# AlgoLab/rs-vgaligner

Hardware: AMD Instinct MI355X
Metric: aligned reads/sec (10 kbp ONT vs HLA graph) (higher is better)
Workload: dtype int32+f64

## Files before the change

rs-vgaligner_amd/csrc/vga_poa_t5.hpp:

```cpp
#pragma once

#include "vga_poa_row.hpp"

__device__ __forceinline__ uint64_t t5_uniform64(uint64_t v)
{
    return ((uint64_t)(uint32_t)__builtin_amdgcn_readfirstlane((int)(v >> 32)) << 32) | (uint32_t)__builtin_amdgcn_readfirstlane((int)(uint32_t)v);
}

#define POA_T5_ARGS_OFFSET 40
__device__ __forceinline__ const poa_t5_args *t5_kargs()
{
    uint32_t off = POA_T5_ARGS_OFFSET;
    asm volatile("" : "+s"(off));
    return (const poa_t5_args *)((const char *)__builtin_amdgcn_kernarg_segment_ptr() + off);
}
template <int NT, bool DEF>
__global__ __launch_bounds__(NT) __attribute__((amdgpu_waves_per_eu(5)))
void k_poa_dp_t5(const poa_prob *__restrict__ probs, const char *__restrict__ queries,
                                                       const uint4 *__restrict__ node_tab, const uint32_t *__restrict__ seq32,
                                                       const uint32_t *__restrict__ preds, const poa_t5_args A)
{
    poa_row *rows = A.rows;
    uint8_t *pool_arg = A.pool;
    const uint32_t lds_cols = t5_own(A.lds_cols), hg_cols = t5_own(A.hg_cols), win_mask = t5_own(A.win_mask);
    enum : uint32_t { ST_CHUNKED = 1u, ST_QPLAIN = 2u, ST_FAILED = 4u, ST_PREV_LDS = 8u, ST_PREV_FAR_USE = 16u };
    uint32_t st = (A.cp.n_slots != 0 ? ST_CHUNKED : 0u) | ST_PREV_LDS;
#define chunked ((st & ST_CHUNKED) != 0)
#define failed ((st & ST_FAILED) != 0)
#define q_plain ((st & ST_QPLAIN) != 0)
#define prev_lds ((st & ST_PREV_LDS) != 0)
#define prev_far_use ((st & ST_PREV_FAR_USE) != 0)
    struct { int match, mismatch, o1, e1, o2, e2, banded; } P = {t5_own(A.P.match), t5_own(A.P.mismatch), A.P.o1, A.P.e1, A.P.o2, A.P.e2, t5_own(A.P.banded)};
    constexpr int NW = NT / 64;
    constexpr int STEP = NT * 4;
    extern __shared__ __attribute__((aligned(16))) uint8_t smem[];
    int4 *sX = (int4 *)smem;
    int4 *sRed = sX + 2 * NW;
    int32_t *edgeW = (int32_t *)(sRed + NW);
    int32_t *sSink = edgeW + 4;
    uint64_t *sChunk = (uint64_t *)(sSink + 4);
    constexpr int HDR = (3 * NW + 1 + 1 + 2) * 16;
    int32_t *Hs = (int32_t *)(smem + HDR);
    uint16_t *Gs = (uint16_t *)(smem + HDR + 4ull * hg_cols);
    uint16_t *Qn = (uint16_t *)(smem + HDR + 6ull * hg_cols);
    const int edge_idx = (int)(edgeW - Hs);

    if (threadIdx.x == 0) A.outs[blockIdx.x].t_begin = __builtin_amdgcn_s_memrealtime();
    if (A.prio) __builtin_amdgcn_s_setprio(3);
    const poa_prob pb = probs[blockIdx.x];
    const int tid = threadIdx.x, lane = tid & 63, wv = __builtin_amdgcn_readfirstlane(tid >> 6);
    const int qlen = t5_own((int)pb.qlen);
    const char *query = queries + pb.q0;
    const uint4 *ntab = node_tab + t5_own(pb.node0);
    const uint32_t *plist = preds + t5_own(pb.pred0);
    const uint32_t *seqw = seq32 + t5_own(pb.seq0 >> 2);
    poa_row *R = rows + t5_own(pb.row0);
    const uint32_t n_nodes = t5_own(pb.n_nodes), ring_rows = t5_own(pb.ring_rows);

    uint8_t *pool = pool_arg;
    uint64_t state_lo = 0, state_hi = 0;
    if (chunked) {
        int got = -1;
        if (!(pb.flags & 1u)) {
            if (tid == 0) {
                got = poa_slot_acquire(A.cp.slot_flag, A.cp.n_slots, blockIdx.x);
                sSink[1] = got;
            }
            __syncthreads();
            got = __builtin_amdgcn_readfirstlane(sSink[1]);
        }
        if (got < 0) {
            if (tid == 0) {
                poa_out &O = A.outs[blockIdx.x];
                O.t_end = O.t_begin; O.cells = 0; O.vcells = 0; O.maxw = 0; O.nops = 0;
                O.score = POA_NEG; O.row = 0; O.status = POA_ST_POOL;
            }
            return;
        }
        __builtin_amdgcn_fence(__ATOMIC_ACQUIRE, "agent");
        pool = nullptr;
        state_lo = (uint64_t)A.cp.state_base + (uint64_t)(uint32_t)got * A.cp.state_size;
        state_hi = state_lo + A.cp.state_size;
    }

    const int o1 = DEF ? 4 : P.o1, e1 = DEF ? 2 : P.e1, o2 = DEF ? 24 : P.o2, e2 = DEF ? 1 : P.e2;
    const int C1 = 4 * (o1 + e1), C2 = 4 * (o2 + e2) + 1;
    const int D1 = 4 * o1, D2 = 4 * o2 + 1;
    const uint32_t g_bias = (uint32_t)(4 * e1 | (4 * e2) << 8) * 0x00010001u;
    const uint32_t e_probe = (uint32_t)((128 - D1) | (128 - D2) << 8) * 0x00010001u;
    const int bw = t5_own((int)pb.w);

    uint32_t own_head = POA_NIL, own_chunks = 0;
    auto alloc = [&](uint64_t &cur, uint32_t &rem, uint32_t bytes_asked, int slot) -> uint64_t {
        const uint32_t bytes = (bytes_asked + 15u) & ~15u;
        if (__builtin_expect(bytes > rem, 0)) {
            if (chunked) {
                if (slot == 0 && bytes <= POA_CHUNK) {
                    const poa_t5_args *ka = t5_kargs();
                    if (tid == 0) {
                        const uint32_t idx = poa_chunk_pop(ka->cp, blockIdx.x);
                        if (idx != POA_NIL) __hip_atomic_store(ka->cp.next + idx, own_head, __ATOMIC_RELAXED, __HIP_MEMORY_SCOPE_AGENT);
                        if (own_chunks == 0) sChunk[3] = idx;
                        sChunk[0] = idx;
                    }
                    __syncthreads();
                    const uint32_t idx = (uint32_t)__builtin_amdgcn_readfirstlane((int)(uint32_t)sChunk[0]);
                    __syncthreads();
                    if (idx == POA_NIL) st |= ST_FAILED;
                    else {
                        own_head = idx;
                        own_chunks++;
                        cur = poa_uniform_u64(poa_chunk_addr(ka->cp, idx));
                        rem = (uint32_t)POA_CHUNK;
                    }
                } else
                    st |= ST_FAILED;
                if (failed) return cur;
            } else {
                const uint64_t need = bytes > POA_CHUNK ? ((uint64_t)bytes + POA_CHUNK - 1) & ~(POA_CHUNK - 1) : POA_CHUNK;
                const poa_t5_args *ka = t5_kargs();
                if (tid == 0) sChunk[slot] = atomicAdd(ka->pool_next, (unsigned long long)need);
                __syncthreads();
                const uint64_t b = t5_uniform64(sChunk[slot]);
                __syncthreads();
                if (b + need > ka->pool_size) st |= ST_FAILED;
                cur = b;
                rem = (uint32_t)need;
            }
        }
        const uint64_t r = cur;
        cur += bytes;
        rem -= bytes;
        return r;
    };

    int non_acgt = 0;
    for (int t = tid; t < (int)(lds_cols / 4); t += NT) {
        uint32_t hw = 0;
#pragma unroll
        for (int k = 0; k < 4; k++) {
            const int j = 4 * t + k;
            uint32_t code = 0;
            if (j >= 1 && j <= qlen) {
                const char ch = query[j - 1];
                code = (ch == 'A' || ch == 'C' || ch == 'G' || ch == 'T') ? 1u << (((uint32_t)ch >> 1) & 3u) : 0u;
                non_acgt |= code == 0;
            }
            hw |= code << (4 * k);
        }
        Qn[t] = (uint16_t)hw;
    }
    if (__builtin_amdgcn_readfirstlane(__syncthreads_or(non_acgt)) == 0) st |= ST_QPLAIN;

    uint64_t dcur = 0, vcur = state_lo, wide_scratch = 0, ring_base = 0;
    uint32_t dend = 0, vendp = (uint32_t)(state_hi - state_lo);
    uint32_t ring_head = 0;
    if (win_mask != 0xFFFFFFFFu) wide_scratch = alloc(vcur, vendp, 2u * 6u * lds_cols, 1);
    {
        const uint64_t maxrow = (6ull * (uint64_t)((qlen + 8) & ~3) + 15ull) & ~15ull;
        if (chunked) {
            ring_base = alloc(vcur, vendp, (uint32_t)(maxrow * (uint64_t)ring_rows), 1);
        } else {
            const uint64_t rb = (maxrow * (uint64_t)ring_rows + POA_CHUNK - 1) & ~(POA_CHUNK - 1);
            if (tid == 0) sChunk[2] = atomicAdd(A.pool_next, (unsigned long long)rb);
            __syncthreads();
            const uint64_t b = t5_uniform64(sChunk[2]);
            if (b + rb > A.pool_size || rb >= (1ull << 32)) st |= ST_FAILED;
            ring_base = b;
        }
    }
    if (tid == 0) { sSink[2] = POA_NEG; sSink[3] = 0; }
    int prev_beg = 0, prev_end = -1;
    uint32_t seq_word = 0, seq_word_idx = 0xFFFFFFFFu;

    for (uint32_t v = 0; v < n_nodes && !failed; v++) {
    const uint4 nt = ntab[v];
    const uint32_t nlen = nt.y & 0xFFFFFFu;
    for (uint32_t tn = 0; tn < nlen && !failed; tn++) {
        asm volatile("" : "+s"(st));
        POA_MARK("row_topo");
        const uint32_t r = nt.x + tn;
        const bool last = tn + 1 == nlen;
        const bool is_sink = last && (nt.z >> 31) != 0;
        const uint32_t ps = nt.w;
        uint32_t gb = 0;
        if (v > 0) {
            const uint32_t bi = r - 1;
            if ((bi & 3u) == 0 || (bi >> 2) != seq_word_idx) { seq_word_idx = bi >> 2; seq_word = seqw[seq_word_idx]; }
            gb = (seq_word >> (8u * (bi & 3u))) & 0xffu;
        }
        const bool simple = r > 0 && prev_lds && (tn > 0 || ((nt.y >> 24) == 1u && ps == r - 1));
        const bool writer = wv == (int)(r % (uint32_t)NW);
        POA_MARK("row_prevmax");
        int prev_lmax = 0, prev_rmax = 0;
        if (r > 0) {
            int4 rw = make_int4(INT32_MIN, INT32_MAX, INT32_MIN, 0);
            if (lane < NW) rw = sRed[lane];
            int b = rw.x, t;
            t = poa_dpp<0x111, 0xf>(INT32_MIN, b); b = t > b ? t : b;
            if (NW > 2) { t = poa_dpp<0x112, 0xf>(INT32_MIN, b); b = t > b ? t : b; }
            if (NW > 4) { t = poa_dpp<0x114, 0xf>(INT32_MIN, b); b = t > b ? t : b; }
            if (NW > 8) { t = poa_dpp<0x118, 0xf>(INT32_MIN, b); b = t > b ? t : b; }
            const int rbest = __builtin_amdgcn_readlane(b, NW - 1);
            const uint64_t tie = __builtin_amdgcn_ballot_w64(rw.x == rbest);
            if (__builtin_expect(__builtin_popcountll(tie) == 1, 1)) {
                const int w1 = __builtin_ctzll(tie);
                prev_lmax = __builtin_amdgcn_readlane(rw.y, w1);
                prev_rmax = __builtin_amdgcn_readlane(rw.z, w1);
            } else {
                int lm = rw.x == rbest ? rw.y : INT32_MAX, rm = rw.x == rbest ? rw.z : INT32_MIN;
                t = poa_dpp<0x111, 0xf>(INT32_MAX, lm); lm = t < lm ? t : lm;
                t = poa_dpp<0x111, 0xf>(INT32_MIN, rm); rm = t > rm ? t : rm;
                if (NW > 2) {
                    t = poa_dpp<0x112, 0xf>(INT32_MAX, lm); lm = t < lm ? t : lm;
                    t = poa_dpp<0x112, 0xf>(INT32_MIN, rm); rm = t > rm ? t : rm;
                }
                if (NW > 4) {
                    t = poa_dpp<0x114, 0xf>(INT32_MAX, lm); lm = t < lm ? t : lm;
                    t = poa_dpp<0x114, 0xf>(INT32_MIN, rm); rm = t > rm ? t : rm;
                }
                if (NW > 8) {
                    t = poa_dpp<0x118, 0xf>(INT32_MAX, lm); lm = t < lm ? t : lm;
                    t = poa_dpp<0x118, 0xf>(INT32_MIN, rm); rm = t > rm ? t : rm;
                }
                prev_lmax = __builtin_amdgcn_readlane(lm, NW - 1);
                prev_rmax = __builtin_amdgcn_readlane(rm, NW - 1);
            }
            if (prev_far_use && writer && lane == 0) { R[r - 1].lmax = prev_lmax; R[r - 1].rmax = prev_rmax; }
        }
        POA_MARK("row_setup");
        const int remain = (int)(nt.z & 0x3fffffffu) + (int)(nlen - 1 - tn);
        int beg, end, np, pbeg = prev_beg, pend = prev_end;
        bool first, single, sp_near;
        uint32_t sp = r - 1;
        uint64_t vpo = 0;
        if (__builtin_expect(simple, 1)) {
            first = tn == 0;
            np = 1; single = true; sp_near = true;
            const int mpl = prev_lmax + 1, mpr = prev_rmax + 1;
            if (!P.banded) { beg = 0; end = qlen; }
            else {
                const int diag = qlen - remain;
                const int lo = mpl < diag ? mpl : diag;
                const int hi = mpr > diag ? mpr : diag;
                beg = lo - bw; if (beg < 0) beg = 0;
                end = hi + bw; if (end > qlen) end = qlen;
            }
        } else {
            first = tn == 0 && v > 0;
            np = v == 0 ? 0 : (tn == 0 ? (int)(nt.y >> 24) : 1);
            bool far = r > 0 && !prev_lds;
            if (first) {
                if (np == 1) far |= ps != r - 1;
                else
                    for (int t = 0; t < np; t++) far |= plist[ps + t] != r - 1;
            }
            single = r > 0 && np == 1;
            sp = first ? ps : r - 1;
            sp_near = sp == r - 1 && prev_lds;
            if (far) __syncthreads();
            int mpl, mpr;
            if (r == 0) { mpl = 0; mpr = 0; }
            else if (!first) { mpl = prev_lmax + 1; mpr = prev_rmax + 1; }
            else {
                mpl = INT32_MAX; mpr = 0;
                for (int t = 0; t < np; t++) {
                    const uint32_t p = np == 1 ? ps : plist[ps + t];
                    int lm, rm;
                    if (p == r - 1) { lm = prev_lmax + 1; rm = prev_rmax + 1; }
                    else {
                        lm = __builtin_amdgcn_readfirstlane(R[p].lmax) + 1;
                        rm = __builtin_amdgcn_readfirstlane(R[p].rmax) + 1;
                    }
                    mpl = lm < mpl ? lm : mpl;
                    mpr = rm > mpr ? rm : mpr;
                }
            }
            if (!P.banded) { beg = 0; end = qlen; }
            else {
                const int diag = qlen - remain;
                const int lo = mpl < diag ? mpl : diag;
                const int hi = mpr > diag ? mpr : diag;
                beg = lo - bw; if (beg < 0) beg = 0;
                end = hi + bw; if (end > qlen) end = qlen;
            }
            if (single && !sp_near) {
                pbeg = __builtin_amdgcn_readfirstlane(R[sp].beg);
                pend = __builtin_amdgcn_readfirstlane(R[sp].end);
                vpo = t5_uniform64(R[sp].voff);
            }
        }
        const int bal = beg & ~3;
        const int W = (end - bal + 1 + 3) & ~3;
        const bool wide = (uint32_t)W + 8u > hg_cols;
        const bool keep = last || wide;
        const uint64_t doff = alloc(dcur, dend, (uint32_t)W * (np > 1 ? 4u : 1u), 0);
        uint64_t voff = 0;
        if (last && !failed) {
            if (r == 0 || (nt.z & 0x40000000u)) voff = chunked ? alloc(dcur, dend, 6u * (uint32_t)W, 0) : alloc(vcur, vendp, 6u * (uint32_t)W, 1);
            else {
                voff = ring_base + (uint64_t)ring_head * ((6u * (uint32_t)((qlen + 8) & ~3) + 15u) & ~15u);
                ring_head = ring_head + 1 == ring_rows ? 0 : ring_head + 1;
            }
        } else if (wide) voff = wide_scratch + (r & 1u) * 6ull * lds_cols;
        if (__builtin_expect(failed, 0)) break;
        if (writer && lane == 0) {
            uint32_t *rec = (uint32_t *)(R + r);
            *(uint4 *)rec = make_uint4((uint32_t)beg, (uint32_t)end, (uint32_t)doff, (uint32_t)(doff >> 32));
            *(uint2 *)(rec + 4) = make_uint2((uint32_t)voff, (uint32_t)(voff >> 32));
            *(HIP_vector_type<uint32_t, 3> *)(rec + 8) = HIP_vector_type<uint32_t, 3>(ps, first ? (uint32_t)np : 0u, keep ? 1u : 0u);
        }
        uint8_t *Vrow = pool + voff;
        uint8_t *drow = pool + doff;
        const uint32_t gd = gb - (uint32_t)'A';
        const bool acgt = gd < 20u && ((0x80045u >> gd) & 1u);
        const int sc_eq = acgt ? P.match : 0, sc_ne = acgt ? -P.mismatch : 0;
        const int gsh = (int)((gb >> 1) & 3u);
        const int ne4t = 4 * sc_ne + 1, mm4 = 4 * (sc_eq - sc_ne);
        const bool staged = !simple && r > 0 && !wide && q_plain;
        if (staged) {
            POA_MARK("row_stage");
            if (chunked) {
                bool no_row = false;
                for (int t = 0; t < np; t++) no_row |= t5_uniform64(R[np == 1 ? sp : plist[ps + t]].voff) == 0;
                if (__builtin_expect(no_row, 0)) st |= ST_FAILED;
            }
            for (int c0 = 0; c0 < W; c0 += STEP) {
                const int c = c0 + 4 * tid;
                const int j0 = bal + c;
                if (j0 <= end && np == 1) {
                    const int bp = __builtin_amdgcn_readfirstlane(R[sp].beg), ep = __builtin_amdgcn_readfirstlane(R[sp].end);
                    const uint64_t vq_off = t5_uniform64(R[sp].voff);
                    const uint8_t *Vq = pool + vq_off;
                    const bool vq_ok = !chunked || vq_off != 0;
                    const int balq = bp & ~3;
                    const int Wq = (ep - balq + 1 + 3) & ~3;
                    const int idx = j0 - balq;
                    int4 hv = make_int4(T4_NEG, T4_NEG, T4_NEG, T4_NEG);
                    uint2 gg = make_uint2(0u, 0u);
                    if (idx >= 0 && idx < Wq && vq_ok) {
                        hv = *(const int4 *)((const int32_t *)Vq + idx);
                        gg = *(const uint2 *)(Vq + 4ll * Wq + 2ll * idx);
                    }
                    const unsigned pspan = (unsigned)(ep - bp);
                    const bool in0 = (unsigned)(j0 - bp) <= pspan, in1 = (unsigned)(j0 + 1 - bp) <= pspan, in2 = (unsigned)(j0 + 2 - bp) <= pspan,
                               in3 = (unsigned)(j0 + 3 - bp) <= pspan;
                    hv.x = in0 ? hv.x : T4_NEG; hv.y = in1 ? hv.y : T4_NEG; hv.z = in2 ? hv.z : T4_NEG; hv.w = in3 ? hv.w : T4_NEG;
                    gg.x = (in0 ? gg.x & 0xffffu : 0u) | (in1 ? gg.x & 0xffff0000u : 0u);
                    gg.y = (in2 ? gg.y & 0xffffu : 0u) | (in3 ? gg.y & 0xffff0000u : 0u);
                    *(int4 *)(Hs + (j0 & win_mask)) = hv;
                    *(uint2 *)(Gs + (j0 & win_mask)) = gg;
                    if (c == 0 && bal > 0) {
                        const int wl = (idx >= 1 && idx - 1 < Wq && vq_ok) ? ((const int32_t *)Vq)[idx - 1] : 0;
                        Hs[(bal - 1) & win_mask] = (unsigned)(j0 - 1 - bp) <= pspan ? wl : T4_NEG;
                    }
                } else if (j0 <= end) {
                    int hm[4], x1[4], x2[4], ah[4], a1[4], a2[4];
                    int hl = T4_NEG, ahl = 0;
#pragma unroll
                    for (int k = 0; k < 4; k++) { hm[k] = T4_NEG; x1[k] = T4_NEG; x2[k] = T4_NEG; ah[k] = 0; a1[k] = 0; a2[k] = 0; }
                    for (int t = 0; t < np; t++) {
                        const uint32_t p = np == 1 ? sp : plist[ps + t];
                        const int bp = __builtin_amdgcn_readfirstlane(R[p].beg), ep = __builtin_amdgcn_readfirstlane(R[p].end);
                        const uint64_t vq_off = t5_uniform64(R[p].voff);
                        const uint8_t *Vq = pool + vq_off;
                        const int balq = bp & ~3;
                        const int Wq = (!chunked || vq_off != 0) ? (ep - balq + 1 + 3) & ~3 : 0;
                        const int idx = j0 - balq;
                        int4 hv = make_int4(0, 0, 0, 0);
                        uint2 gg = make_uint2(0u, 0u);
                        if (idx >= 0 && idx < Wq) {
                            hv = *(const int4 *)((const int32_t *)Vq + idx);
                            gg = *(const uint2 *)(Vq + 4ll * Wq + 2ll * idx);
                        }
                        int wl = (idx >= 1 && idx - 1 < Wq) ? ((const int32_t *)Vq)[idx - 1] : 0;
                        const unsigned pspan = (unsigned)(ep - bp);
                        const int hj[4] = {hv.x, hv.y, hv.z, hv.w};
                        const uint32_t g16[4] = {gg.x & 0xffffu, gg.x >> 16, gg.y & 0xffffu, gg.y >> 16};
#pragma unroll
                        for (int k = 0; k < 4; k++) {
                            if ((unsigned)(j0 + k - bp) <= pspan) {
                                const int h = hj[k], c1 = h - (int)(g16[k] & 255u), c2 = h - (int)(g16[k] >> 8);
                                if (h > hm[k]) { hm[k] = h; ah[k] = t; }
                                if (c1 > x1[k]) { x1[k] = c1; a1[k] = t; }
                                if (c2 > x2[k]) { x2[k] = c2; a2[k] = t; }
                            }
                        }
                        if (j0 >= 1 && (unsigned)(j0 - 1 - bp) <= pspan && wl > hl) { hl = wl; ahl = t; }
                    }
                    const int4 hq = make_int4(hm[0], hm[1], hm[2], hm[3]);
                    uint32_t gv[4];
#pragma unroll
                    for (int k = 0; k < 4; k++) gv[k] = (uint32_t)(hm[k] - x1[k]) | ((uint32_t)(hm[k] - x2[k]) << 8);
                    *(int4 *)(Hs + (j0 & win_mask)) = hq;
                    *(uint2 *)(Gs + (j0 & win_mask)) = make_uint2(gv[0] | (gv[1] << 16), gv[2] | (gv[3] << 16));
                    if (c == 0 && bal > 0) Hs[(bal - 1) & win_mask] = hl;
                    if (np > 1) {
                        *(uint32_t *)(drow + (uint64_t)W + c) = (uint32_t)ahl | ((uint32_t)ah[0] << 8) | ((uint32_t)ah[1] << 16) | ((uint32_t)ah[2] << 24);
                        *(uint32_t *)(drow + 2ull * W + c) = (uint32_t)a1[0] | ((uint32_t)a1[1] << 8) | ((uint32_t)a1[2] << 16) | ((uint32_t)a1[3] << 24);
                        *(uint32_t *)(drow + 3ull * W + c) = (uint32_t)a2[0] | ((uint32_t)a2[1] << 8) | ((uint32_t)a2[2] << 16) | ((uint32_t)a2[3] << 24);
                    }
                }
            }
            POA_LDS_BARRIER();
            pbeg = bal > 0 ? bal - 1 : 0;
            pend = bal + W - 1;
        }
        const uint8_t *Vp = pool + vpo;
        const int balp = pbeg & ~3;

        POA_MARK("row_steps");
        enum : uint32_t { F_SINGLE = 1u, F_NEAR = 2u, F_PLAIN = 4u, F_WIDE = 8u, F_KEEP = 16u, F_SINK = 32u, F_MULTI = 64u, F_SRC = 128u };
        const uint32_t rowf = (single ? F_SINGLE : 0u) | (sp_near ? F_NEAR : 0u) | (q_plain ? F_PLAIN : 0u) | (wide ? F_WIDE : 0u) |
                              (keep ? F_KEEP : 0u) | (is_sink ? F_SINK : 0u) | (np > 1 ? F_MULTI : 0u) | (r == 0 ? F_SRC : 0u);
        int best = INT32_MIN, lpos = beg, rpos = beg;
        const bool hot = (simple || staged) && !wide && q_plain;
        const int rlim = end < pend ? end : pend;
        auto run_steps = [&](auto hot_c) __attribute__((always_inline)) {
        constexpr bool HOT = decltype(hot_c)::value;
        int carry1 = POA_IDENT, carry2 = POA_IDENT, left1 = POA_IDENT, left2 = POA_IDENT;
        int next_left = 0;
        int buf = 0;
        for (int c0 = 0; c0 < W; c0 += STEP, buf ^= 1) {
            uint32_t f = HOT ? (rowf & (F_KEEP | F_SINK)) : rowf;
            asm volatile("" : "+s"(f));
            if (HOT) f |= F_SINGLE | F_NEAR | F_PLAIN;
            const int c = c0 + 4 * tid;
            const int j0 = bal + c;
            const bool lane_act = j0 <= end;
            const int jw0 = bal + c0 + 256 * wv, jw1 = jw0 + 255;
            const bool wave_act = jw0 <= end;
            int d_lp = jw0 - beg, d_rp = rlim - jw1, d_lq = (jw0 > beg ? jw0 : beg) - pbeg - 1;
            asm volatile("" : "+s"(d_lp), "+s"(d_rp), "+s"(d_lq));
            const uint32_t e_lp = (uint32_t)d_lp >> 31;
            const uint32_t e_rp = (uint32_t)d_rp >> 31;
            const uint32_t e_lq = (uint32_t)d_lq >> 31;
            const bool lp = e_lp != 0, rp = e_rp != 0, lq = e_lq != 0;
            int htt[4], ht4[4], e1t[4], e2t[4], pmeta[4];
            int agg1 = POA_IDENT, agg2 = POA_IDENT, alast1 = POA_IDENT, alast2 = POA_IDENT;
#pragma unroll
            for (int k = 0; k < 4; k++) { htt[k] = T4_NEG + 2; ht4[k] = T4_NEG; e1t[k] = T4_NEG + 1; e2t[k] = T4_NEG; pmeta[k] = 0; }
            uint32_t qn = 0u;
            if (wave_act) qn = (uint32_t)Qn[j0 >> 2];
            const bool fastw = HOT ? wave_act
                                   : (f & (F_SINGLE | F_PLAIN)) == (F_SINGLE | F_PLAIN) && wave_act && (!lq || (f & F_NEAR)) && (!rp || ((f & F_NEAR) && end <= pend + 1));
            const int base1 = 4 * e1 * j0, base2 = 4 * e2 * j0;
        if constexpr (HOT) POA_MARK("hot_p1_fast"); else POA_MARK("p1_fast");
            if (__builtin_expect(fastw, 1)) {
                int4 hv;
                uint2 gg;
                int hprev;
                if constexpr (HOT) {
                    hv = *(const int4 *)(Hs + (j0 & win_mask));
                    gg = *(const uint2 *)(Gs + (j0 & win_mask));
                    int left0;
                    if (wv == 0 && c0 > 0) left0 = next_left;
                    else left0 = Hs[(jw0 > 0 ? jw0 - 1 : 0) & (int)win_mask];
                    if (wv == 0 && c0 + STEP < W) next_left = Hs[(jw0 + STEP - 1) & (int)win_mask];
                    hprev = t4_shr1_mov(hv.w, left0);
                } else if (__builtin_expect((f & F_NEAR) != 0, 1)) {
                    hv = *(const int4 *)(Hs + (j0 & win_mask));
                    gg = *(const uint2 *)(Gs + (j0 & win_mask));
                    if (tid == NT - 1) edgeW[buf] = hv.w;
                    {
                        const bool edge = tid == 0 && c0 > 0;
                        int w = Hs[edge ? edge_idx + (buf ^ 1) : ((j0 > 0 ? j0 - 1 : 0) & win_mask)];
                        asm volatile("" : "+v"(w));
                        hprev = w;
                    }
                } else {
                    const int Wp = (pend - balp + 1 + 3) & ~3;
                    const int idx = j0 - balp;
                    hv = *(const int4 *)((const int32_t *)Vp + idx);
                    gg = *(const uint2 *)(Vp + 4ll * Wp + 2ll * idx);
                    hprev = ((const int32_t *)Vp)[idx > 0 ? idx - 1 : 0];
                    asm volatile("" : "+v"(hv.x), "+v"(hv.y), "+v"(hv.z), "+v"(hv.w), "+v"(gg.x), "+v"(gg.y), "+v"(hprev));
                }
                auto phase1 = [&](auto edge_c) {
                    constexpr bool EDGE = decltype(edge_c)::value;
                    int hj[4] = {hv.x, hv.y, hv.z, hv.w};
                    int ga = (int)gg.x, gbb = (int)gg.y;
                    if constexpr (EDGE) {
                        if (rp) {
#pragma unroll
                            for (int k = 0; k < 4; k++) hj[k] = j0 + k > pend ? T4_NEG : hj[k];
                            ga = j0 > pend ? 0 : (j0 + 1 > pend ? (ga & 0xffff) : ga);
                            gbb = j0 + 2 > pend ? 0 : (j0 + 3 > pend ? (gbb & 0xffff) : gbb);
                        }
                        if (lq) {
#pragma unroll
                            for (int k = 0; k < 4; k++) hj[k] = j0 + k < pbeg ? T4_NEG : hj[k];
                            ga = j0 + 1 < pbeg ? 0 : (j0 < pbeg ? (int)((uint32_t)ga & 0xffff0000u) : ga);
                            gbb = j0 + 3 < pbeg ? 0 : (j0 + 2 < pbeg ? (int)((uint32_t)gbb & 0xffff0000u) : gbb);
                        }
                    }
                    const uint32_t eqb = qn >> gsh;
                    int hp = hprev;
                    if constexpr (EDGE && HOT) {
                        if (rp) hp = j0 - 1 > pend ? T4_NEG : hp;
                    }
#pragma unroll
                    for (int k = 0; k < 4; k++) {
                        const int g = k < 2 ? ga : gbb;
                        const int ev1 = (k & 1) ? t4_sub_byte<2>(hj[k], g) : t4_sub_byte<0>(hj[k], g);
                        const int ev2 = (k & 1) ? t4_sub_byte<3>(hj[k], g) : t4_sub_byte<1>(hj[k], g);
                        int m = (int)__umul24(__builtin_amdgcn_ubfe(eqb, 4u * k, 1u), (uint32_t)mm4) + (hp + ne4t);
                        if constexpr (EDGE) {
                            if (lq) m = j0 + k - 1 < pbeg ? T4_NEG + 2 : m;
                        }
                        const int h = t4_max3(m, ev1, ev2);
                        htt[k] = h;
                        ht4[k] = h & ~3;
                        e1t[k] = ev1;
                        e2t[k] = ev2;
                        hp = hj[k];
                    }
                    if constexpr (EDGE) {
                        if (lp) {
#pragma unroll
                            for (int k = 0; k < 4; k++) ht4[k] = j0 + k < beg ? POA_IDENT : ht4[k];
                        }
                    }
                    const int r11 = ht4[1] + 4 * e1, r12 = ht4[2] + 8 * e1, r13 = ht4[3] + 12 * e1;
                    const int r21 = ht4[1] + 4 * e2, r22 = ht4[2] + 8 * e2, r23 = ht4[3] + 12 * e2;
                    const int a1 = t4_max3(ht4[0], r11, r12), a2 = t4_max3(ht4[0], r21, r22);
                    agg1 = (a1 > r13 ? a1 : r13) + base1;
                    agg2 = (a2 > r23 ? a2 : r23) + base2;
                    alast1 = r13 + base1;
                    alast2 = r23 + base2;
                };
                if (__builtin_expect((e_lp | e_rp | e_lq) != 0, 0)) phase1(std::true_type{});
                else phase1(std::false_type{});
        if constexpr (HOT) POA_MARK("hot_p1_lean"); else POA_MARK("p1_lean");
            } else if (wave_act && (f & F_SINGLE)) {
                int pbeg_ = pbeg, pend_ = pend, beg_ = beg, end_ = end, balp_ = balp, gsh_ = gsh;
                asm volatile("" : "+s"(pbeg_), "+s"(pend_), "+s"(beg_), "+s"(end_), "+s"(balp_), "+s"(gsh_));
                const int pbeg = pbeg_, pend = pend_, beg = beg_, end = end_, balp = balp_, gsh = gsh_;
                const unsigned span = (unsigned)(end - beg), pspan = (unsigned)(pend - pbeg);
                int hj[4], wm0;
                uint32_t g16[4];
                if (f & F_NEAR) {
                    const int4 hv = *(const int4 *)(Hs + (j0 & win_mask));
                    const uint2 gg = *(const uint2 *)(Gs + (j0 & win_mask));
                    hj[0] = hv.x; hj[1] = hv.y; hj[2] = hv.z; hj[3] = hv.w;
                    g16[0] = gg.x & 0xffffu; g16[1] = gg.x >> 16; g16[2] = gg.y & 0xffffu; g16[3] = gg.y >> 16;
                    if (tid == NT - 1) edgeW[buf] = hj[3];
                    const bool edge = tid == 0 && c0 > 0;
                    int w = Hs[edge ? edge_idx + (buf ^ 1) : ((j0 > 0 ? j0 - 1 : 0) & win_mask)];
                    asm volatile("" : "+v"(w));
                    wm0 = w;
                } else {
                    const int idx = j0 - balp;
                    const int Wp = (pend - balp + 1 + 3) & ~3;
                    int4 hv = make_int4(0, 0, 0, 0);
                    uint2 gg = make_uint2(0u, 0u);
                    if (idx >= 0 && idx < Wp) {
                        hv = *(const int4 *)((const int32_t *)Vp + idx);
                        gg = *(const uint2 *)(Vp + 4ll * Wp + 2ll * idx);
                    }
                    wm0 = (idx >= 1 && idx - 1 < Wp) ? ((const int32_t *)Vp)[idx - 1] : 0;
                    asm volatile("" : "+v"(hv.x), "+v"(hv.y), "+v"(hv.z), "+v"(hv.w), "+v"(gg.x), "+v"(gg.y), "+v"(wm0));
                    hj[0] = hv.x; hj[1] = hv.y; hj[2] = hv.z; hj[3] = hv.w;
                    g16[0] = gg.x & 0xffffu; g16[1] = gg.x >> 16; g16[2] = gg.y & 0xffffu; g16[3] = gg.y >> 16;
                }
                bool inprev = j0 >= 1 && (unsigned)(j0 - 1 - pbeg) <= pspan;
#pragma unroll
                for (int k = 0; k < 4; k++) {
                    const int j = j0 + k;
                    const bool inj = (unsigned)(j - pbeg) <= pspan;
                    const bool actk = (unsigned)(j - beg) <= span;
                    const int qc = (int)((qn >> (4 * k)) & 15u);
                    const int s = ((qc >> gsh) & 1) ? sc_eq : (qc == 0 ? 0 : sc_ne);
                    const int wm = k == 0 ? wm0 : hj[k - 1];
                    const int m = inprev ? wm + 4 * s + 1 : T4_NEG + 2;
                    const int ev1 = inj ? hj[k] - (int)(g16[k] & 255u) : T4_NEG + 1;
                    const int ev2 = inj ? hj[k] - (int)(g16[k] >> 8) : T4_NEG;
                    const int h = t4_max3(m, ev1, ev2);
                    htt[k] = h;
                    ht4[k] = h & ~3;
                    e1t[k] = ev1;
                    e2t[k] = ev2;
                    const int a1 = actk ? ht4[k] + 4 * e1 * j : POA_IDENT, a2 = actk ? ht4[k] + 4 * e2 * j : POA_IDENT;
                    agg1 = a1 > agg1 ? a1 : agg1;
                    agg2 = a2 > agg2 ? a2 : agg2;
                    if (k == 3) { alast1 = a1; alast2 = a2; }
                    inprev = inj;
                }
        if constexpr (HOT) POA_MARK("hot_p1_general"); else POA_MARK("p1_general");
            } else if (wave_act) {
                int beg_ = beg, end_ = end, gsh_ = gsh;
                asm volatile("" : "+s"(beg_), "+s"(end_), "+s"(gsh_));
                const int beg = beg_, end = end_, gsh = gsh_;
                const unsigned span = (unsigned)(end - beg);
                if (f & F_SRC) {
#pragma unroll
                    for (int k = 0; k < 4; k++) { ht4[k] = (j0 + k == 0) ? 0 : T4_NEG; htt[k] = ht4[k] + 2; }
                } else if (lane_act) {
                    int m[4], ev1[4], ev2[4];
#pragma unroll
                    for (int k = 0; k < 4; k++) { m[k] = T4_NEG + 2; ev1[k] = T4_NEG + 1; ev2[k] = T4_NEG; }
                    for (int t = 0; t < np; t++) {
                        const uint32_t p = plist[ps + t];
                        int hj[4], wm0 = 0;
                        uint32_t g16[4];
                        int bp, ep;
                        if (p == r - 1 && prev_lds) {
                            bp = prev_beg; ep = prev_end;
                            const int4 hv = *(const int4 *)(Hs + (j0 & win_mask));
                            const uint2 gg = *(const uint2 *)(Gs + (j0 & win_mask));
                            hj[0] = hv.x; hj[1] = hv.y; hj[2] = hv.z; hj[3] = hv.w;
                            g16[0] = gg.x & 0xffffu; g16[1] = gg.x >> 16; g16[2] = gg.y & 0xffffu; g16[3] = gg.y >> 16;
                            if (tid == NT - 1) edgeW[buf] = hj[3];
                            const bool edge = tid == 0 && c0 > 0;
                            int w = Hs[edge ? edge_idx + (buf ^ 1) : ((j0 > 0 ? j0 - 1 : 0) & win_mask)];
                            asm volatile("" : "+v"(w));
                            wm0 = w;
                        } else {
                            bp = __builtin_amdgcn_readfirstlane(R[p].beg);
                            ep = __builtin_amdgcn_readfirstlane(R[p].end);
                            const uint64_t vo = R[p].voff;
                            const uint64_t vos = ((uint64_t)(uint32_t)__builtin_amdgcn_readfirstlane((int)(vo >> 32)) << 32) |
                                                 (uint32_t)__builtin_amdgcn_readfirstlane((int)(uint32_t)vo);
                            const uint8_t *Vq = pool + vos;
                            const int balq = bp & ~3;
                            const int Wq = (ep - balq + 1 + 3) & ~3;
                            const int idx = j0 - balq;
                            int4 hv = make_int4(0, 0, 0, 0);
                            uint2 gg = make_uint2(0u, 0u);
                            if (idx >= 0 && idx < Wq) {
                                hv = *(const int4 *)((const int32_t *)Vq + idx);
                                gg = *(const uint2 *)(Vq + 4ll * Wq + 2ll * idx);
                            }
                            wm0 = (idx >= 1 && idx - 1 < Wq) ? ((const int32_t *)Vq)[idx - 1] : 0;
                            asm volatile("" : "+v"(hv.x), "+v"(hv.y), "+v"(hv.z), "+v"(hv.w), "+v"(gg.x), "+v"(gg.y), "+v"(wm0));
                            hj[0] = hv.x; hj[1] = hv.y; hj[2] = hv.z; hj[3] = hv.w;
                            g16[0] = gg.x & 0xffffu; g16[1] = gg.x >> 16; g16[2] = gg.y & 0xffffu; g16[3] = gg.y >> 16;
                        }
                        const unsigned pspan = (unsigned)(ep - bp);
#pragma unroll
                        for (int k = 0; k < 4; k++) {
                            const int j = j0 + k;
                            const bool actk = (unsigned)(j - beg) <= span;
                            const int qc = (int)((qn >> (4 * k)) & 15u);
                            const int s = ((qc >> gsh) & 1) ? sc_eq : (qc == 0 ? 0 : sc_ne);
                            const int wm = k == 0 ? wm0 : hj[k - 1];
                            if (actk && j >= 1 && (unsigned)(j - 1 - bp) <= pspan) {
                                const int cnd = wm + 4 * s + 1;
                                if (cnd > m[k]) { m[k] = cnd; pmeta[k] = (pmeta[k] & ~255) | t; }
                            }
                            if (actk && (unsigned)(j - bp) <= pspan) {
                                const int c1 = hj[k] - (int)(g16[k] & 255u);
                                if (c1 > ev1[k]) { ev1[k] = c1; pmeta[k] = (pmeta[k] & ~0xff00) | (t << 8); }
                                const int c2 = hj[k] - (int)(g16[k] >> 8);
                                if (c2 > ev2[k]) { ev2[k] = c2; pmeta[k] = (pmeta[k] & ~0xff0000) | (t << 16); }
                            }
                        }
                    }
#pragma unroll
                    for (int k = 0; k < 4; k++) {
                        const int h = t4_max3(m[k], ev1[k], ev2[k]);
                        htt[k] = h;
                        ht4[k] = h & ~3;
                        e1t[k] = ev1[k];
                        e2t[k] = ev2[k];
                    }
                }
#pragma unroll
                for (int k = 0; k < 4; k++) {
                    const int j = j0 + k;
                    const bool actk = (unsigned)(j - beg) <= span;
                    const int a1 = actk ? ht4[k] + 4 * e1 * j : POA_IDENT, a2 = actk ? ht4[k] + 4 * e2 * j : POA_IDENT;
                    agg1 = a1 > agg1 ? a1 : agg1;
                    agg2 = a2 > agg2 ? a2 : agg2;
                    if (k == 3) { alast1 = a1; alast2 = a2; }
                }
            }
        if constexpr (HOT) POA_MARK("hot_scan"); else POA_MARK("scan");
            int i1 = POA_IDENT, i2 = POA_IDENT;
            if (wave_act) {
                i1 = poa_wave_scan_max(agg1);
                i2 = poa_wave_scan_max(agg2);
            }
            if (lane == 63) sX[buf * NW + wv] = make_int4(i1, i2, alast1, alast2);
            POA_LDS_BARRIER();
        if constexpr (HOT) POA_MARK("hot_exchange"); else POA_MARK("exchange");
            int pre1 = carry1, pre2 = carry2, pl1 = left1, pl2 = left2;
            {
                const bool more = c0 + STEP < W;
                if ((wave_act && wv > 0) || more) {
                    int4 x = make_int4(POA_IDENT, POA_IDENT, POA_IDENT, POA_IDENT);
                    if (lane < NW) x = sX[buf * NW + lane];
                    int s1 = x.x, s2 = x.y, t;
                    t = poa_dpp<0x111, 0xf>(INT32_MIN, s1); s1 = t > s1 ? t : s1;
                    t = poa_dpp<0x111, 0xf>(INT32_MIN, s2); s2 = t > s2 ? t : s2;
                    if (NW > 2) {
                        t = poa_dpp<0x112, 0xf>(INT32_MIN, s1); s1 = t > s1 ? t : s1;
                        t = poa_dpp<0x112, 0xf>(INT32_MIN, s2); s2 = t > s2 ? t : s2;
                    }
                    if (NW > 4) {
                        t = poa_dpp<0x114, 0xf>(INT32_MIN, s1); s1 = t > s1 ? t : s1;
                        t = poa_dpp<0x114, 0xf>(INT32_MIN, s2); s2 = t > s2 ? t : s2;
                    }
                    if (NW > 8) {
                        t = poa_dpp<0x118, 0xf>(INT32_MIN, s1); s1 = t > s1 ? t : s1;
                        t = poa_dpp<0x118, 0xf>(INT32_MIN, s2); s2 = t > s2 ? t : s2;
                    }
                    if (wv > 0) {
                        const int a = __builtin_amdgcn_readlane(s1, wv - 1), b = __builtin_amdgcn_readlane(s2, wv - 1);
                        pre1 = a > pre1 ? a : pre1;
                        pre2 = b > pre2 ? b : pre2;
                        pl1 = __builtin_amdgcn_readlane(x.z, wv - 1);
                        pl2 = __builtin_amdgcn_readlane(x.w, wv - 1);
                    }
                    if (more) {
                        const int a = __builtin_amdgcn_readlane(s1, NW - 1), b = __builtin_amdgcn_readlane(s2, NW - 1);
                        carry1 = a > carry1 ? a : carry1;
                        carry2 = b > carry2 ? b : carry2;
                        left1 = __builtin_amdgcn_readlane(x.z, NW - 1);
                        left2 = __builtin_amdgcn_readlane(x.w, NW - 1);
                    }
                }
            }
            if (wave_act) {
                const int run1_ = t4_shr1_max(i1, pre1), run2_ = t4_shr1_max(i2, pre2);
                const int la1_ = t4_shr1_mov(alast1, pl1), la2_ = t4_shr1_mov(alast2, pl2);
        if constexpr (HOT) POA_MARK("hot_p2_fast"); else POA_MARK("p2_fast");
                if (__builtin_expect(fastw, 1)) {
                    auto phase2 = [&](auto edge_c) {
                        constexpr bool EDGE = decltype(edge_c)::value;
                        int R1 = run1_ - base1, R2 = run2_ - base2, L1 = la1_ - base1, L2 = la2_ - base2;
                        int h4[4];
                        int dirq = 0, ga = 0, gbb = 0;
#pragma unroll
                        for (int k = 0; k < 4; k++) {
                            const int f1 = R1 - (4 * (o1 + e1 * k) - 1), f2 = R2 - 4 * (o2 + e2 * k);
                            const int hh = t4_max3(ht4[k] | 3, f1, f2);
                            const int h = (hh & ~3) | 1;
                            h4[k] = h;
                            int acc = (hh << 2) | (htt[k] & 3);
                            const int u1 = h - e1t[k], u2 = h - e2t[k];
                            if (k == 0) { t5_min_byte<0>(ga, u1, D1); t5_min_byte<1>(ga, u2, D2); }
                            if (k == 1) { t5_min_byte<2>(ga, u1, D1); t5_min_byte<3>(ga, u2, D2); }
                            if (k == 2) { t5_min_byte<0>(gbb, u1, D1); t5_min_byte<1>(gbb, u2, D2); }
                            if (k == 3) { t5_min_byte<2>(gbb, u1, D1); t5_min_byte<3>(gbb, u2, D2); }
                            t4_flag_ne(acc, R1, L1);
                            if (k == 0) t4_flag_ne_dep<0>(dirq, acc, R2, L2);
                            if (k == 1) t4_flag_ne_dep<1>(dirq, acc, R2, L2);
                            if (k == 2) t4_flag_ne_dep<2>(dirq, acc, R2, L2);
                            if (k == 3) t4_flag_ne_dep<3>(dirq, acc, R2, L2);
                            L1 = ht4[k] + 4 * e1 * k; L2 = ht4[k] + 4 * e2 * k;
                            R1 = L1 > R1 ? L1 : R1;
                            R2 = L2 > R2 ? L2 : R2;
                        }
                        {
                            const uint32_t ya = (uint32_t)ga + e_probe, yb = ((uint32_t)gbb + e_probe) >> 1;
                            const uint32_t e8 = (ya & 0x80808080u) | (yb & ~0x80808080u);
                            dirq = (int)((e8 & 0xC0C0C0C0u) | ((uint32_t)dirq & ~0xC0C0C0C0u));
                            ga = (int)((uint32_t)ga + g_bias);
                            gbb = (int)((uint32_t)gbb + g_bias);
                        }
                        {
                            int hb[4] = {h4[0], h4[1], h4[2], h4[3]};
                            if constexpr (EDGE) {
#pragma unroll
                                for (int k = 0; k < 4; k++) hb[k] = j0 + k > end ? INT32_MIN : hb[k];
                            }
                            const int m3 = t4_max3(hb[0], hb[1], hb[2]);
                            const int m4 = m3 > hb[3] ? m3 : hb[3];
                            if (m4 >= best) {
                                const int kf = hb[0] == m4 ? 0 : (hb[1] == m4 ? 1 : (hb[2] == m4 ? 2 : 3));
                                const int kl = hb[3] == m4 ? 3 : (hb[2] == m4 ? 2 : (hb[1] == m4 ? 1 : 0));
                                if (m4 > best) { best = m4; lpos = j0 + kf; }
                                rpos = j0 + kl;
                            }
                        }
                        if (__builtin_expect((f & F_SINK) != 0, 0)) {
                            const int kq = qlen - j0;
#pragma unroll
                            for (int k = 0; k < 4; k++)
                                if (kq == k) sSink[0] = h4[k];
                        }
                        if (!EDGE || j0 <= end) {
                            const int4 hq = make_int4(h4[0], h4[1], h4[2], h4[3]);
                            const uint2 gq = make_uint2((uint32_t)ga, (uint32_t)gbb);
                            if (!(f & F_WIDE)) {
                                *(int4 *)(Hs + (j0 & win_mask)) = hq;
                                *(uint2 *)(Gs + (j0 & win_mask)) = gq;
                            }
                            *(uint32_t *)(drow + c) = (uint32_t)dirq;
                            if (f & F_KEEP) {
                                *(int4 *)((int32_t *)Vrow + c) = hq;
                                *(uint2 *)(Vrow + 4ll * W + 2ll * c) = gq;
                            }
                        }
                    };
                    if (__builtin_expect((e_lp | e_rp) != 0, 0)) phase2(std::true_type{});
                    else phase2(std::false_type{});
        if constexpr (HOT) POA_MARK("hot_p2_slow"); else POA_MARK("p2_slow");
                } else if (lane_act) {
                    int beg_ = beg, end_ = end;
                    asm volatile("" : "+s"(beg_), "+s"(end_));
                    const int beg = beg_;
                    const unsigned span = (unsigned)(end_ - beg_);
                    int run1 = run1_, run2 = run2_, la1 = la1_, la2 = la2_;
                    int h4[4];
                    uint32_t g16[4], codev[4];
#pragma unroll
                    for (int k = 0; k < 4; k++) {
                        const int j = j0 + k;
                        const bool actk = (unsigned)(j - beg) <= span;
                        const int f1 = run1 - 4 * (o1 + e1 * j) + 1, f2 = run2 - 4 * (o2 + e2 * j);
                        const int hh = t4_max3(ht4[k] | 3, f1, f2);
                        const int h = (hh & ~3) | 1;
                        h4[k] = h;
                        const uint32_t t1 = (uint32_t)((h + 4 * e1) - e1t[k]), t2 = (uint32_t)((h + 4 * e2) - e2t[k]);
                        const uint32_t G1 = t1 < (uint32_t)C1 ? t1 : (uint32_t)C1, G2 = t2 < (uint32_t)C2 ? t2 : (uint32_t)C2;
                        g16[k] = G1 | (G2 << 8);
                        codev[k] = (((uint32_t)(hh & 3) << 4) | ((uint32_t)(htt[k] & 3) << 2) | (run1 != la1 ? 2u : 0u) | (run2 != la2 ? 1u : 0u)) << (8 * k);
                        codev[k] |= ((t1 >= (uint32_t)C1 ? 1u : 0u) | (t2 >= (uint32_t)C2 ? 256u : 0u)) << (16 * (k & 1) + (k < 2 ? 7 : 6));
                        const int hb = actk ? h : INT32_MIN;
                        if (hb > best) { best = hb; lpos = j; rpos = j; }
                        else if (actk && hb == best) rpos = j;
                        const int a1 = actk ? ht4[k] + 4 * e1 * j : POA_IDENT, a2 = actk ? ht4[k] + 4 * e2 * j : POA_IDENT;
                        run1 = a1 > run1 ? a1 : run1;
                        run2 = a2 > run2 ? a2 : run2;
                        la1 = actk ? a1 : la1; la2 = actk ? a2 : la2;
                    }
                    if (__builtin_expect((f & F_SINK) != 0, 0)) {
                        const int kq = qlen - j0;
#pragma unroll
                        for (int k = 0; k < 4; k++)
                            if (kq == k) sSink[0] = h4[k];
                    }
                    const int Wl = (end_ - bal + 1 + 3) & ~3;
                    {
                        const int4 hq = make_int4(h4[0], h4[1], h4[2], h4[3]);
                        const uint2 gq = make_uint2(g16[0] | (g16[1] << 16), g16[2] | (g16[3] << 16));
                        if (!(f & F_WIDE)) {
                            *(int4 *)(Hs + (j0 & win_mask)) = hq;
                            *(uint2 *)(Gs + (j0 & win_mask)) = gq;
                        }
                        *(uint32_t *)(drow + c) = codev[0] | codev[1] | codev[2] | codev[3];
                        if (f & F_KEEP) {
                            *(int4 *)((int32_t *)Vrow + c) = hq;
                            *(uint2 *)(Vrow + 4ll * Wl + 2ll * c) = gq;
                        }
                        if (__builtin_expect((f & F_MULTI) != 0, 0)) {
                            *(uint32_t *)(drow + (uint64_t)Wl + c) = (uint32_t)(pmeta[0] & 255) | ((uint32_t)(pmeta[1] & 255) << 8) | ((uint32_t)(pmeta[2] & 255) << 16) | ((uint32_t)(pmeta[3] & 255) << 24);
                            *(uint32_t *)(drow + 2ull * Wl + c) = (uint32_t)((pmeta[0] >> 8) & 255) | ((uint32_t)((pmeta[1] >> 8) & 255) << 8) | ((uint32_t)((pmeta[2] >> 8) & 255) << 16) | ((uint32_t)((pmeta[3] >> 8) & 255) << 24);
                            *(uint32_t *)(drow + 3ull * Wl + c) = (uint32_t)((pmeta[0] >> 16) & 255) | ((uint32_t)((pmeta[1] >> 16) & 255) << 8) | ((uint32_t)((pmeta[2] >> 16) & 255) << 16) | ((uint32_t)((pmeta[3] >> 16) & 255) << 24);
                        }
                    }
                }
            }
        if constexpr (HOT) POA_MARK("hot_step_end"); else POA_MARK("step_end");
        }
        };
        if (__builtin_expect(hot, 1)) run_steps(std::true_type{});
        else run_steps(std::false_type{});
        POA_MARK("row_reduce");
        {
            const int wb = __builtin_amdgcn_readlane(poa_wave_scan_max(best), 63);
            const bool mine = best == wb;
            const uint64_t tie = __builtin_amdgcn_ballot_w64(mine);
            int *red = (int *)(sRed + wv);
            if (__builtin_expect(__builtin_popcountll(tie) == 1, 1)) {
                if (mine) { red[0] = best; red[1] = lpos; red[2] = rpos; }
            } else {
                int lm = mine ? lpos : INT32_MAX, rm = mine ? rpos : INT32_MIN;
                lm = poa_wave_scan_min(lm);
                rm = poa_wave_scan_max(rm);
                if (lane == 63) { red[0] = wb; red[1] = lm; red[2] = rm; }
            }
        }
        POA_LDS_BARRIER();
        POA_MARK("row_end");
        if (__builtin_expect(is_sink, 0) && tid == 0) {
            const int val = (qlen >= beg && qlen <= end) ? sSink[0] >> 2 : POA_NEG;
            if (sSink[3] == 0 || val > sSink[2]) { sSink[2] = val; sSink[3] = (int)r + 1; }
        }
        prev_beg = beg; prev_end = end;
        st = (st & ~(ST_PREV_LDS | ST_PREV_FAR_USE)) | (wide ? 0u : ST_PREV_LDS) | (last ? ST_PREV_FAR_USE : 0u);
    }
    }
    POA_MARK("epilogue");
    __syncthreads();
    if (tid >= 64) return;
    const poa_t5_args E = *t5_kargs();
    const poa_prob pe = E.probs[blockIdx.x];
    poa_out &O = E.outs[blockIdx.x];
    int status = POA_ST_OK;
    uint32_t start_row = 0;
    int sink_best = POA_NEG;
    if (failed) status = POA_ST_POOL;
    else {
        sink_best = __builtin_amdgcn_readfirstlane(sSink[2]);
        const int sr = __builtin_amdgcn_readfirstlane(sSink[3]);
        start_row = sr ? (uint32_t)(sr - 1) : 0u;
        status = (sr != 0 && sink_best > POA_NEG / 2) ? POA_ST_OK : POA_ST_NOALN;
        const poa_row *Rr = E.rows + pe.row0;
        uint64_t cells = 0, vcells = 0;
        int maxw = 0;
        for (uint32_t r = (uint32_t)lane; r <= pe.N; r += 64) {
            const int b = Rr[r].beg, e = Rr[r].end, kp = Rr[r].base;
            const int W = (e - (b & ~3) + 1 + 3) & ~3;
            maxw = W > maxw ? W : maxw;
            if (r > 0) cells += (uint64_t)(e - b + 1);
            if (kp) vcells += (uint64_t)(e - b + 1);
        }
        for (int sh = 32; sh > 0; sh >>= 1) {
            cells += __shfl_down(cells, sh);
            vcells += __shfl_down(vcells, sh);
            const int m2 = __shfl_down(maxw, sh);
            maxw = m2 > maxw ? m2 : maxw;
        }
        if (tid == 0) { O.cells = cells; O.vcells = vcells; O.maxw = (uint32_t)maxw; }
    }
    if (tid == 0) {
        if (failed) { O.cells = 0; O.vcells = 0; O.maxw = 0; }
        O.score = failed ? POA_NEG : sink_best;
        O.row = start_row;
        O.status = status;
    }
    if (E.tb_ops) {
        uint8_t *pool_e = E.cp.n_slots ? nullptr : E.pool;
        poa_traceback_wave<2>(*(tb_lds *)(smem + HDR), tid, pe, E.rows, E.preds, pool_e, O, E.tb_ops, E.tb_orow, 0, status, start_row);
    }
    if (tid == 0) {
        O.t_end = __builtin_amdgcn_s_memrealtime();
        if (E.cp.n_slots) {
            const uint32_t state_slot = (uint32_t)sSink[1];
            if (own_head != POA_NIL) poa_chunk_push(E.cp, blockIdx.x, own_head, (uint32_t)sChunk[3]);
            const uint64_t state_lo = (uint64_t)E.cp.state_base + (uint64_t)state_slot * E.cp.state_size;
            (void)atomicAdd(E.pool_next, (unsigned long long)own_chunks * POA_CHUNK + (vcur - state_lo));
            __builtin_amdgcn_fence(__ATOMIC_RELEASE, "agent");
            (void)atomicExch(&E.cp.slot_flag[state_slot], 0u);
        }
    }
}
#undef chunked
#undef failed
#undef q_plain
#undef prev_lds
#undef prev_far_use
```

Measured before the change: 10590.

## Split predecessor staging into single/multi paths with wave-uniform interior fast path and LDS reuse

Staging of predecessor rows now branches once on the predecessor count. The single-predecessor path hoists the row metadata out of the column loop and uses pbeg/pend/vpo instead of re-reading R. Both paths add a wave-uniform interior check that skips the per-lane bounds masking when a whole 256-column wave chunk lies inside the predecessor span. The multi-predecessor path takes the immediately preceding row straight from the LDS window rather than reloading it from global memory, at the cost of extra LDS barriers per column chunk and added code size and register pressure.

```diff
diff --git a/rs-vgaligner_amd/csrc/vga_poa_t5.hpp b/rs-vgaligner_amd/csrc/vga_poa_t5.hpp
--- a/rs-vgaligner_amd/csrc/vga_poa_t5.hpp
+++ b/rs-vgaligner_amd/csrc/vga_poa_t5.hpp
@@ -325,80 +325,149 @@
                 for (int t = 0; t < np; t++) no_row |= t5_uniform64(R[np == 1 ? sp : plist[ps + t]].voff) == 0;
                 if (__builtin_expect(no_row, 0)) st |= ST_FAILED;
             }
-            for (int c0 = 0; c0 < W; c0 += STEP) {
-                const int c = c0 + 4 * tid;
-                const int j0 = bal + c;
-                if (j0 <= end && np == 1) {
-                    const int bp = __builtin_amdgcn_readfirstlane(R[sp].beg), ep = __builtin_amdgcn_readfirstlane(R[sp].end);
-                    const uint64_t vq_off = t5_uniform64(R[sp].voff);
-                    const uint8_t *Vq = pool + vq_off;
-                    const bool vq_ok = !chunked || vq_off != 0;
-                    const int balq = bp & ~3;
-                    const int Wq = (ep - balq + 1 + 3) & ~3;
+            if (np == 1) {
+                const int bp = pbeg, ep = pend;
+                const uint8_t *Vq = pool + vpo;
+                const bool vq_ok = !chunked || vpo != 0;
+                const int balq = bp & ~3;
+                const int Wq = (ep - balq + 1 + 3) & ~3;
+                const unsigned pspan = (unsigned)(ep - bp);
+                for (int c0 = 0; c0 < W; c0 += STEP) {
+                    const int c = c0 + 4 * tid;
+                    const int j0 = bal + c;
+                    const int jw0 = bal + c0 + 256 * wv;
+                    int d_in = (jw0 - 1 - bp) | (ep - 255 - jw0);
+                    asm volatile("" : "+s"(d_in));
+                    if (j0 > end) continue;
                     const int idx = j0 - balq;
-                    int4 hv = make_int4(T4_NEG, T4_NEG, T4_NEG, T4_NEG);
-                    uint2 gg = make_uint2(0u, 0u);
-                    if (idx >= 0 && idx < Wq && vq_ok) {
-                        hv = *(const int4 *)((const int32_t *)Vq + idx);
-                        gg = *(const uint2 *)(Vq + 4ll * Wq + 2ll * idx);
-                    }
-                    const unsigned pspan = (unsigned)(ep - bp);
-                    const bool in0 = (unsigned)(j0 - bp) <= pspan, in1 = (unsigned)(j0 + 1 - bp) <= pspan, in2 = (unsigned)(j0 + 2 - bp) <= pspan,
-                               in3 = (unsigned)(j0 + 3 - bp) <= pspan;
-                    hv.x = in0 ? hv.x : T4_NEG; hv.y = in1 ? hv.y : T4_NEG; hv.z = in2 ? hv.z : T4_NEG; hv.w = in3 ? hv.w : T4_NEG;
-                    gg.x = (in0 ? gg.x & 0xffffu : 0u) | (in1 ? gg.x & 0xffff0000u : 0u);
-                    gg.y = (in2 ? gg.y & 0xffffu : 0u) | (in3 ? gg.y & 0xffff0000u : 0u);
-                    *(int4 *)(Hs + (j0 & win_mask)) = hv;
-                    *(uint2 *)(Gs + (j0 & win_mask)) = gg;
-                    if (c == 0 && bal > 0) {
-                        const int wl = (idx >= 1 && idx - 1 < Wq && vq_ok) ? ((const int32_t *)Vq)[idx - 1] : 0;
-                        Hs[(bal - 1) & win_mask] = (unsigned)(j0 - 1 - bp) <= pspan ? wl : T4_NEG;
-                    }
-                } else if (j0 <= end) {
+                    if (d_in >= 0 && vq_ok) {
+                        *(int4 *)(Hs + (j0 & win_mask)) = *(const int4 *)((const int32_t *)Vq + idx);
+                        *(uint2 *)(Gs + (j0 & win_mask)) = *(const uint2 *)(Vq + 4ll * Wq + 2ll * idx);
+                        if (c == 0 && bal > 0) Hs[(bal - 1) & win_mask] = ((const int32_t *)Vq)[idx - 1];
+                    } else {
+                        int4 hv = make_int4(T4_NEG, T4_NEG, T4_NEG, T4_NEG);
+                        uint2 gg = make_uint2(0u, 0u);
+                        if (idx >= 0 && idx < Wq && vq_ok) {
+                            hv = *(const int4 *)((const int32_t *)Vq + idx);
+                            gg = *(const uint2 *)(Vq + 4ll * Wq + 2ll * idx);
+                        }
+                        const bool in0 = (unsigned)(j0 - bp) <= pspan, in1 = (unsigned)(j0 + 1 - bp) <= pspan, in2 = (unsigned)(j0 + 2 - bp) <= pspan,
+                                   in3 = (unsigned)(j0 + 3 - bp) <= pspan;
+                        hv.x = in0 ? hv.x : T4_NEG; hv.y = in1 ? hv.y : T4_NEG; hv.z = in2 ? hv.z : T4_NEG; hv.w = in3 ? hv.w : T4_NEG;
+                        gg.x = (in0 ? gg.x & 0xffffu : 0u) | (in1 ? gg.x & 0xffff0000u : 0u);
+                        gg.y = (in2 ? gg.y & 0xffffu : 0u) | (in3 ? gg.y & 0xffff0000u : 0u);
+                        *(int4 *)(Hs + (j0 & win_mask)) = hv;
+                        *(uint2 *)(Gs + (j0 & win_mask)) = gg;
+                        if (c == 0 && bal > 0) {
+                            const int wl = (idx >= 1 && idx - 1 < Wq && vq_ok) ? ((const int32_t *)Vq)[idx - 1] : 0;
+                            Hs[(bal - 1) & win_mask] = (unsigned)(j0 - 1 - bp) <= pspan ? wl : T4_NEG;
+                        }
+                    }
+                }
+            } else {
+                struct pred_rec { int bp, ep; uint64_t voff; };
+                auto read_rec = [&](uint32_t p) {
+                    return pred_rec{__builtin_amdgcn_readfirstlane(R[p].beg), __builtin_amdgcn_readfirstlane(R[p].end), t5_uniform64(R[p].voff)};
+                };
+                int t_up = -1;
+                for (int t = 0; t < np; t++)
+                    if (plist[ps + t] == r - 1 && prev_lds) t_up = t;
+                int up_left = 0;
+                for (int c0 = 0; c0 < W; c0 += STEP) {
+                    const int c = c0 + 4 * tid;
+                    const int j0 = bal + c;
+                    const int jw0 = bal + c0 + 256 * wv;
+                    const bool lane_act = j0 <= end;
+                    int4 uh = make_int4(0, 0, 0, 0);
+                    uint2 ug = make_uint2(0u, 0u);
+                    int uw = 0;
+                    if (t_up >= 0) {
+                        if (lane_act) {
+                            uh = *(const int4 *)(Hs + (j0 & win_mask));
+                            ug = *(const uint2 *)(Gs + (j0 & win_mask));
+                            uw = Hs[(j0 > 0 ? j0 - 1 : 0) & win_mask];
+                            if (tid == 0) {
+                                if (c0 > 0) uw = up_left;
+                                if (c0 + STEP < W) up_left = Hs[(j0 + STEP - 1) & win_mask];
+                            }
+                        }
+                        POA_LDS_BARRIER();
+                    }
                     int hm[4], x1[4], x2[4], ah[4], a1[4], a2[4];
                     int hl = T4_NEG, ahl = 0;
 #pragma unroll
                     for (int k = 0; k < 4; k++) { hm[k] = T4_NEG; x1[k] = T4_NEG; x2[k] = T4_NEG; ah[k] = 0; a1[k] = 0; a2[k] = 0; }
                     for (int t = 0; t < np; t++) {
-                        const uint32_t p = np == 1 ? sp : plist[ps + t];
-                        const int bp = __builtin_amdgcn_readfirstlane(R[p].beg), ep = __builtin_amdgcn_readfirstlane(R[p].end);
-                        const uint64_t vq_off = t5_uniform64(R[p].voff);
-                        const uint8_t *Vq = pool + vq_off;
-                        const int balq = bp & ~3;
-                        const int Wq = (!chunked || vq_off != 0) ? (ep - balq + 1 + 3) & ~3 : 0;
-                        const int idx = j0 - balq;
-                        int4 hv = make_int4(0, 0, 0, 0);
-                        uint2 gg = make_uint2(0u, 0u);
-                        if (idx >= 0 && idx < Wq) {
-                            hv = *(const int4 *)((const int32_t *)Vq + idx);
-                            gg = *(const uint2 *)(Vq + 4ll * Wq + 2ll * idx);
-                        }
-                        int wl = (idx >= 1 && idx - 1 < Wq) ? ((const int32_t *)Vq)[idx - 1] : 0;
-                        const unsigned pspan = (unsigned)(ep - bp);
-                        const int hj[4] = {hv.x, hv.y, hv.z, hv.w};
-                        const uint32_t g16[4] = {gg.x & 0xffffu, gg.x >> 16, gg.y & 0xffffu, gg.y >> 16};
-#pragma unroll
-                        for (int k = 0; k < 4; k++) {
-                            if ((unsigned)(j0 + k - bp) <= pspan) {
-                                const int h = hj[k], c1 = h - (int)(g16[k] & 255u), c2 = h - (int)(g16[k] >> 8);
-                                if (h > hm[k]) { hm[k] = h; ah[k] = t; }
-                                if (c1 > x1[k]) { x1[k] = c1; a1[k] = t; }
-                                if (c2 > x2[k]) { x2[k] = c2; a2[k] = t; }
+                        if (lane_act) {
+                            const bool up = t == t_up;
+                            pred_rec q = {prev_beg, prev_end, 0};
+                            if (!up) q = read_rec(plist[ps + t]);
+                            const int bp = q.bp, ep = q.ep;
+                            const uint64_t vq_off = q.voff;
+                            const uint8_t *Vq = pool + vq_off;
+                            const int balq = bp & ~3;
+                            const int Wq = (!chunked || vq_off != 0) ? (ep - balq + 1 + 3) & ~3 : 0;
+                            const int idx = j0 - balq;
+                            int d_in = (jw0 - 1 - bp) | (ep - 255 - jw0);
+                            asm volatile("" : "+s"(d_in));
+                            int4 hv = uh;
+                            uint2 gg = ug;
+                            int wl = uw;
+                            if (d_in >= 0 && (up || Wq != 0)) {
+                                if (!up) {
+                                    hv = *(const int4 *)((const int32_t *)Vq + idx);
+                                    gg = *(const uint2 *)(Vq + 4ll * Wq + 2ll * idx);
+                                    wl = ((const int32_t *)Vq)[idx - 1];
+                                }
+                                const int hj[4] = {hv.x, hv.y, hv.z, hv.w};
+                                const uint32_t g16[4] = {gg.x & 0xffffu, gg.x >> 16, gg.y & 0xffffu, gg.y >> 16};
+#pragma unroll
+                                for (int k = 0; k < 4; k++) {
+                                    const int h = hj[k], c1 = h - (int)(g16[k] & 255u), c2 = h - (int)(g16[k] >> 8);
+                                    if (h > hm[k]) { hm[k] = h; ah[k] = t; }
+                                    if (c1 > x1[k]) { x1[k] = c1; a1[k] = t; }
+                                    if (c2 > x2[k]) { x2[k] = c2; a2[k] = t; }
+                                }
+                                if (wl > hl) { hl = wl; ahl = t; }
+                            } else {
+                                if (!up) {
+                                    hv = make_int4(0, 0, 0, 0);
+                                    gg = make_uint2(0u, 0u);
+                                    if (idx >= 0 && idx < Wq) {
+                                        hv = *(const int4 *)((const int32_t *)Vq + idx);
+                                        gg = *(const uint2 *)(Vq + 4ll * Wq + 2ll * idx);
+                                    }
+                                    wl = (idx >= 1 && idx - 1 < Wq) ? ((const int32_t *)Vq)[idx - 1] : 0;
+                                }
+                                const unsigned pspan = (unsigned)(ep - bp);
+                                const int hj[4] = {hv.x, hv.y, hv.z, hv.w};
+                                const uint32_t g16[4] = {gg.x & 0xffffu, gg.x >> 16, gg.y & 0xffffu, gg.y >> 16};
+#pragma unroll
+                                for (int k = 0; k < 4; k++) {
+                                    if ((unsigned)(j0 + k - bp) <= pspan) {
+                                        const int h = hj[k], c1 = h - (int)(g16[k] & 255u), c2 = h - (int)(g16[k] >> 8);
+                                        if (h > hm[k]) { hm[k] = h; ah[k] = t; }
+                                        if (c1 > x1[k]) { x1[k] = c1; a1[k] = t; }
+                                        if (c2 > x2[k]) { x2[k] = c2; a2[k] = t; }
+                                    }
+                                }
+                                if (j0 >= 1 && (unsigned)(j0 - 1 - bp) <= pspan && wl > hl) { hl = wl; ahl = t; }
                             }
                         }
-                        if (j0 >= 1 && (unsigned)(j0 - 1 - bp) <= pspan && wl > hl) { hl = wl; ahl = t; }
-                    }
-                    const int4 hq = make_int4(hm[0], hm[1], hm[2], hm[3]);
-                    uint32_t gv[4];
-#pragma unroll
-                    for (int k = 0; k < 4; k++) gv[k] = (uint32_t)(hm[k] - x1[k]) | ((uint32_t)(hm[k] - x2[k]) << 8);
-                    *(int4 *)(Hs + (j0 & win_mask)) = hq;
-                    *(uint2 *)(Gs + (j0 & win_mask)) = make_uint2(gv[0] | (gv[1] << 16), gv[2] | (gv[3] << 16));
-                    if (c == 0 && bal > 0) Hs[(bal - 1) & win_mask] = hl;
-                    if (np > 1) {
-                        *(uint32_t *)(drow + (uint64_t)W + c) = (uint32_t)ahl | ((uint32_t)ah[0] << 8) | ((uint32_t)ah[1] << 16) | ((uint32_t)ah[2] << 24);
-                        *(uint32_t *)(drow + 2ull * W + c) = (uint32_t)a1[0] | ((uint32_t)a1[1] << 8) | ((uint32_t)a1[2] << 16) | ((uint32_t)a1[3] << 24);
-                        *(uint32_t *)(drow + 3ull * W + c) = (uint32_t)a2[0] | ((uint32_t)a2[1] << 8) | ((uint32_t)a2[2] << 16) | ((uint32_t)a2[3] << 24);
+                    }
+                    if (lane_act) {
+                        const int4 hq = make_int4(hm[0], hm[1], hm[2], hm[3]);
+                        uint32_t gv[4];
+#pragma unroll
+                        for (int k = 0; k < 4; k++) gv[k] = (uint32_t)(hm[k] - x1[k]) | ((uint32_t)(hm[k] - x2[k]) << 8);
+                        *(int4 *)(Hs + (j0 & win_mask)) = hq;
+                        *(uint2 *)(Gs + (j0 & win_mask)) = make_uint2(gv[0] | (gv[1] << 16), gv[2] | (gv[3] << 16));
+                        if (c == 0 && bal > 0) Hs[(bal - 1) & win_mask] = hl;
+                        if (np > 1) {
+                            *(uint32_t *)(drow + (uint64_t)W + c) = (uint32_t)ahl | ((uint32_t)ah[0] << 8) | ((uint32_t)ah[1] << 16) | ((uint32_t)ah[2] << 24);
+                            *(uint32_t *)(drow + 2ull * W + c) = (uint32_t)a1[0] | ((uint32_t)a1[1] << 8) | ((uint32_t)a1[2] << 16) | ((uint32_t)a1[3] << 24);
+                            *(uint32_t *)(drow + 3ull * W + c) = (uint32_t)a2[0] | ((uint32_t)a2[1] << 8) | ((uint32_t)a2[2] << 16) | ((uint32_t)a2[3] << 24);
+                        }
                     }
                 }
             }
```

Result: slower. 10490 (-1.0%).
